# wsntxxn/AudioCaption

Measured on AMD Instinct MI355X. Metric: clips/sec (10 s @ 32 kHz) encode+greedy-decode, Cnn14_Rnn-Trm, higher is better.
Workload: dtype bf16x3

## Files before the change

### audiocaption_amd/csrc/conv3x3_block1_w4.hip

```cpp
#include <stdlib.h>
#include <string.h>
#include <type_traits>

#include "ac_common.h"
#include "ac_drop.h"
#include "ac_wino43.h"

namespace {

#ifndef B1_RING
#define B1_RING 3
#endif

#ifndef B1_RING_MFC
#define B1_RING_MFC 6
#endif
#ifndef B1_SGB_MEM
#define B1_SGB_MEM 0x0b0
#endif
#ifndef B1_SGB
#define B1_SGB 0
#endif
#ifndef B1_KO
#define B1_KO 0
#endif
#ifdef B1_CLK
__device__ unsigned long long b1_clk[8];
#endif

typedef unsigned u32x4 __attribute__((ext_vector_type(4)));

struct B1Params {
  const float* in;
  const float* w1;
  const float* sc1;
  const float* sh1;
  const void* wpk;
  const float* scale;
  const float* shift;
  float* out;
  int rows_total, Hp, H;
  int tiles;
  const int* clip_frames;
  int need_mul, need_add;
  Drop drop;
};

constexpr int B1_W = 64, B1_COLP = 3;
constexpr int B1_HALF = (((B1_W + 2) * B1_COLP * 16 + 127) / 128) * 128 + 64;
constexpr int B1_PLANE = 2 * B1_HALF;
constexpr int B1_VBUF = 12 * B1_PLANE;
constexpr int B1_WT = 2 * B1_VBUF;
constexpr int B1_LDS = B1_WT + 4096;
static_assert(B1_LDS <= 160 * 1024, "LDS");

template <int FORM, bool DROP>
__global__ __launch_bounds__(256, 1) void block1_w4_kernel(B1Params p) {
  constexpr bool FUSED = FORM == 1, MFC = FORM == 2;
  constexpr int HALF = B1_HALF, PLANE = B1_PLANE, VBUF = B1_VBUF, COLP = B1_COLP;
  extern __shared__ __attribute__((aligned(128))) unsigned char dsm_raw[];
  unsigned char* sV = dsm_raw;
  float* wt = (float*)(dsm_raw + B1_WT);
  const int tid = threadIdx.x;
  const int lane = tid & 63;
  const int wave = __builtin_amdgcn_readfirstlane(tid >> 6);
  const int half = lane >> 5;
  const int cg = wave & 1, wq = wave >> 1;
  const int nblk = (int)gridDim.x;

  auto tile_live = [&](int t) { return w4_rows_live(8 * t, 8, p.rows_total, p.Hp, p.H, p.clip_frames, p.need_mul, p.need_add); };
  auto zero_tile = [&](int t) {
    const f32x4 z = {0.f, 0.f, 0.f, 0.f};
    float* o = p.out + (size_t)t * 4 * 32 * 64;
    const long left = ((long)p.rows_total / 2 - 4L * t) * 32 * 64;
#pragma unroll
    for (int k = 0; k < 8; ++k) {
      const int i = (k * 256 + tid) * 4;
      if (i < left) *(f32x4*)(o + i) = z;
    }
  };
  auto next_live = [&](int t) {
    t += nblk;
    while (t < p.tiles && !tile_live(t)) { zero_tile(t); t += nblk; }
    return t;
  };
  int tile = next_live((int)blockIdx.x - nblk);
  if (tile >= p.tiles) return;

  {
    constexpr int NZ = 2 * 24 * 2 * COLP;
    const f32x4 z = {0.f, 0.f, 0.f, 0.f};
    for (int i = tid; i < NZ; i += 256) {
      const int slot = i % COLP, col = (i / COLP) & 1, hh = (i / (2 * COLP)) % 24, b = i / (48 * COLP);
      *(f32x4*)(sV + b * VBUF + hh * HALF + ((col ? B1_W + 1 : 0) * COLP + slot) * 16) = z;
    }
    if (FUSED) {
      for (int i = tid; i < 64 * 12; i += 256) {
        const int ch = i / 12, k = i % 12;
        wt[i] = k < 9 ? p.w1[ch * 9 + k] : (k == 9 ? p.sc1[ch] : (k == 10 ? p.sh1[ch] : 0.f));
      }
    }
    if (MFC && tid < 128) {
      const int ct = tid >> 6, l = tid & 63, ch = 32 * ct + (l & 31), h = l >> 5;
      const float sc = p.sc1[ch];
      f32x4 v[2];
#pragma unroll
      for (int q = 0; q < 8; ++q) {
        const int ky = 2 * h + q / 4, kx = q % 4;
        float w = 0.f;
        if (ky < 3 && kx < 3) w = p.w1[ch * 9 + ky * 3 + kx] * sc;
        if (ky == 3 && kx == 0) w = p.sh1[ch];
        v[q / 4][q % 4] = w;
      }
      u32x2 hi0, lo0, hi1, lo1;
      split_bf16x4(v[0], hi0, lo0);
      split_bf16x4(v[1], hi1, lo1);
      unsigned* dst = (unsigned*)(dsm_raw + B1_WT) + (ct * 2 * 64 + l) * 4;
      dst[0] = hi0.x; dst[1] = hi0.y; dst[2] = hi1.x; dst[3] = hi1.y;
      dst[256] = lo0.x; dst[257] = lo0.y; dst[258] = lo1.x; dst[259] = lo1.y;
    }
  }

  unsigned pb[2];
  {
    const int i = lane & 31;
#pragma unroll
    for (int m = 0; m < 2; ++m) pb[m] = (unsigned)(half * HALF + ((32 * m + i) * COLP + wq) * 16);
  }
  const int cq = tid & 3, scol = tid >> 2;
  unsigned lofs[2];
#pragma unroll
  for (int j = 0; j < 2; ++j) lofs[j] = (unsigned)((cq >> 1) * HALF + ((scol + 1) * COLP + j) * 16 + (cq & 1) * 8);

  const __amdgpu_buffer_rsrc_t rw = __builtin_amdgcn_make_buffer_rsrc((void*)p.wpk, 0, 4 * 18 * 4096, 0x00020000);
  const unsigned wvoff = (unsigned)(cg * 2048 + lane * 16);
  auto w_load = [&](int s, int gi, bf16x8 (&w)[2]) {
    const unsigned soff = (unsigned)((s & 3) * 18 + gi) * 4096u;
    w[0] = __builtin_bit_cast(bf16x8, __builtin_amdgcn_raw_buffer_load_b128(rw, wvoff, soff, 0));
    w[1] = __builtin_bit_cast(bf16x8, __builtin_amdgcn_raw_buffer_load_b128(rw, wvoff + 1024u, soff, 0));
  };

  const size_t in_elems = (size_t)p.rows_total * 64 * (FORM ? 1 : 64);
  const __amdgpu_buffer_rsrc_t rx = __builtin_amdgcn_make_buffer_rsrc(
      (void*)p.in, 0, (int)(in_elems * 4 < 0x7fffffffull ? in_elems * 4 : 0x7fffffffull), 0x00020000);

  auto load_x = [&](int t, float (&x)[12][3]) {
    const int cl = scol == 0 ? 0 : scol - 1, cr = scol == 63 ? 63 : scol + 1;
#pragma unroll
    for (int j = 0; j < 12; ++j) {
      const int gr = 8 * t - 2 + j;
      const unsigned off = (unsigned)(gr * 256);
      const float a = __builtin_bit_cast(float, __builtin_amdgcn_raw_buffer_load_b32(rx, off + (unsigned)(cl * 4), 0, 0));
      const float b = __builtin_bit_cast(float, __builtin_amdgcn_raw_buffer_load_b32(rx, off + (unsigned)(scol * 4), 0, 0));
      const float c = __builtin_bit_cast(float, __builtin_amdgcn_raw_buffer_load_b32(rx, off + (unsigned)(cr * 4), 0, 0));
      x[j][0] = scol == 0 ? 0.f : a;
      x[j][1] = b;
      x[j][2] = scol == 63 ? 0.f : c;
    }
  };
  float touch = 0.f;
  auto touch_x = [&](int t) {
    if (tid < 24) {
      const unsigned off = (unsigned)(((8 * t - 2) * 64 + tid * 32) * 4);
      touch = __builtin_bit_cast(float, __builtin_amdgcn_raw_buffer_load_b32(rx, off, 0, 0));
    }
  };
  auto row_mask = [&](int t) {
    unsigned m = 0;
    for (int r = 0; r < 10; ++r) {
      const int gr = 8 * t - 1 + r;
      if (gr >= 0 && gr < p.rows_total && (gr % p.Hp) < p.H) m |= 1u << r;
    }
    return m;
  };

  f32x16 acc[6][2];
  constexpr int RING = MFC && !DROP ? B1_RING_MFC : B1_RING, AH = RING - 1;
  bf16x8 wr[RING][2];
  bf16x8 af[2][2][2];
  float xc[12][3];
  unsigned mask_c = 0;
  f32x4 c1[10];
  f32x4 c1b[10];
  f32x4 w1r[4][3];

  auto conv1_row = [&](const float (&x)[12][3], unsigned mask, int r) {
    f32x4 y;
#pragma unroll
    for (int e = 0; e < 4; ++e) {
      float a = 0.f;
#pragma unroll
      for (int t = 0; t < 9; ++t) a = fmaf(x[r + t / 3][t % 3], w1r[e][t / 4][t % 4], a);
      y[e] = fmaxf(fmaf(a, w1r[e][2][1], w1r[e][2][2]), 0.f);
    }
    const f32x4 z = {0.f, 0.f, 0.f, 0.f};
    return (mask >> r) & 1u ? y : z;
  };
  auto taps_load = [&](int s) {
#pragma unroll
    for (int e = 0; e < 4; ++e)
#pragma unroll
      for (int k = 0; k < 3; ++k) w1r[e][k] = *(const f32x4*)(wt + ((s & 3) * 16 + cq * 4 + e) * 12 + 4 * k);
  };
  auto rows_request = [&](int t, int s, f32x4 (&dst)[10]) {
#pragma unroll
    for (int r = 0; r < 10; ++r) {
      const long gr = 8L * t - 1 + r;
      const unsigned off = (unsigned)(((gr * 64 + scol) * 64 + (s & 3) * 16 + cq * 4) * 4);
      dst[r] = __builtin_bit_cast(f32x4, __builtin_amdgcn_raw_buffer_load_b128(rx, off, 0, 0));
    }
  };
  auto piece = [&](unsigned char* buf, const f32x4 (&d)[10], int j, int pos) {
    const f32x4 v = w4_transform(pos, d[4 * j], d[4 * j + 1], d[4 * j + 2], d[4 * j + 3], d[4 * j + 4], d[4 * j + 5]);
    u32x2 hi, lo;
    split_bf16x4(v, hi, lo);
    unsigned char* dst = buf + lofs[j] + (2 * pos) * PLANE;
    *(u32x2*)dst = hi;
    *(u32x2*)(dst + PLANE) = lo;
  };
  auto stage_unit = [&](unsigned char* buf, int gi, int S, const float (&x)[12][3], unsigned mask, f32x4 (&d)[10]) {
    constexpr int ROW_AT[16] = {0, 1, 2, 3, 4, -1, -1, 5, -1, 6, 7, 8, -1, -1, 9, -1};
    constexpr int PIECE_AT[16] = {-1, -1, -1, -1, -1, 0, 2, -1, 4, -1, -1, -1, 6, 8, -1, 10};
    if (gi >= 16 || (B1_KO & 1)) return;
    if (FUSED && gi == 0) taps_load(S);
    if (FUSED && ROW_AT[gi] >= 0) d[ROW_AT[gi]] = conv1_row(x, mask, ROW_AT[gi]);
    if (PIECE_AT[gi] >= 0) {
      piece(buf, d, PIECE_AT[gi] / 6, PIECE_AT[gi] % 6);
      piece(buf, d, (PIECE_AT[gi] + 1) / 6, (PIECE_AT[gi] + 1) % 6);
    }
  };
  auto a_load = [&](const unsigned char* buf, int gi, bf16x8 (&a)[2][2]) {
    const int kx = gi / 6, q = gi % 6;
    const unsigned char* vh = buf + (2 * q) * PLANE + kx * COLP * 16;
#pragma unroll
    for (int m = 0; m < 2; ++m) {
      a[m][0] = *(const bf16x8*)(vh + pb[m]);
      a[m][1] = *(const bf16x8*)(vh + PLANE + pb[m]);
    }
  };

  const int m1 = wave & 1, j1 = wave >> 1;
  const int c1col = 32 * m1 + (lane & 31);
  unsigned lofs1[2];
#pragma unroll
  for (int gh = 0; gh < 2; ++gh) lofs1[gh] = (unsigned)(gh * HALF + ((c1col + 1) * COLP + j1) * 16 + half * 8);
  f32x4 xr[7];
  u32x2 rph[7], rpl[7];
  f32x4 d1[4][6];
  f32x16 c1a[2];
  bf16x8 a1h, a1l;
  auto x_request = [&](int t) {
    const int row0 = 8 * t - 2 + 4 * j1 + 2 * half;
    const int cadj = c1col == 0 ? 0 : c1col - 1;
#pragma unroll
    for (int k = 0; k < 7; ++k)
      xr[k] = __builtin_bit_cast(f32x4, __builtin_amdgcn_raw_buffer_load_b128(rx, (unsigned)(((row0 + k) * 64 + cadj) * 4), 0, 0));
  };
  auto x_convert = [&](int k) {
    const bool first = c1col == 0, last = c1col == 63;
    if (B1_KO & 64) {
      rph[k].x = __builtin_bit_cast(unsigned, xr[k][0]); rph[k].y = __builtin_bit_cast(unsigned, xr[k][1]);
      rpl[k].x = __builtin_bit_cast(unsigned, xr[k][2]); rpl[k].y = __builtin_bit_cast(unsigned, xr[k][3]);
      return;
    }
    const float e0 = first ? 0.f : xr[k][0], e1 = first ? xr[k][0] : xr[k][1];
    const float e2 = last ? 0.f : (first ? xr[k][1] : xr[k][2]);
    const unsigned h0 = cvt_pk_bf16(e0, e1), h1 = cvt_pk_bf16(e2, 0.f);
    const float f0 = __builtin_bit_cast(float, h0 << 16), f1 = __builtin_bit_cast(float, h0 & 0xffff0000u);
    const float f2 = __builtin_bit_cast(float, h1 << 16);
    rph[k].x = h0; rph[k].y = h1;
    rpl[k].x = cvt_pk_bf16(e0 - f0, e1 - f1);
    rpl[k].y = cvt_pk_bf16(e2 - f2, 0.f);
  };
  auto a1_load = [&](int ct) {
    const unsigned char* t = dsm_raw + B1_WT + (ct * 2 * 64 + lane) * 16;
    a1h = *(const bf16x8*)t;
    a1l = *(const bf16x8*)(t + 1024);
  };
  auto c1_mfma = [&](int which, int r) {
    f32x16& a = c1a[r & 1];
    if (B1_KO & 32) {
      if (which == 0) {
#pragma unroll
        for (int k = 0; k < 16; ++k) a[k] = __builtin_bit_cast(float, rph[r].x);
      } else {
        a[which] += __builtin_bit_cast(float, rpl[r + 1].y);
      }
      return;
    }
    if (which == 0) {
      const u32x4 bl = {rpl[r].x, rpl[r].y, half ? 0u : rpl[r + 1].x, half ? 0u : rpl[r + 1].y};
      f32x16 z;
#pragma unroll
      for (int k = 0; k < 16; ++k) z[k] = 0.f;
      a = __builtin_amdgcn_mfma_f32_32x32x16_bf16(a1h, __builtin_bit_cast(bf16x8, bl), z, 0, 0, 0);
    } else {
      const u32x4 bh = {rph[r].x, rph[r].y, half ? 0x3f80u : rph[r + 1].x, half ? 0u : rph[r + 1].y};
      a = __builtin_amdgcn_mfma_f32_32x32x16_bf16(which == 1 ? a1l : a1h, __builtin_bit_cast(bf16x8, bh), a, 0, 0, 0);
    }
  };
  auto c1_post = [&](int r, unsigned mask) {
    const float cap = (mask >> (4 * j1 + r)) & 1u ? __builtin_inff() : 0.f;
#pragma unroll
    for (int g = 0; g < 4; ++g)
#pragma unroll
      for (int e = 0; e < 4; ++e) d1[g][r][e] = __builtin_amdgcn_fmed3f(c1a[r & 1][4 * g + e], 0.f, cap);
  };
  auto piece1 = [&](unsigned char* buf, int g, int pos) {
    const f32x4 v = w4_transform(pos, d1[g][0], d1[g][1], d1[g][2], d1[g][3], d1[g][4], d1[g][5]);
    u32x2 hi, lo;
    split_bf16x4(v, hi, lo);
    unsigned char* dst = buf + lofs1[g & 1] + (2 * pos) * PLANE;
    if (B1_KO & 8) {
      asm volatile("" :: "v"(hi), "v"(lo), "v"(dst));
      return;
    }
    *(u32x2*)dst = hi;
    *(u32x2*)(dst + PLANE) = lo;
  };
  auto stage_a = [&](unsigned char* buf, int gi, int ct, unsigned mask) {
    if (B1_KO & 1) return;
    if (gi == 0) a1_load(ct);
    if (gi == 0) {
#pragma unroll
      for (int k = 0; k < 7; ++k) x_convert(k);
    }
    if (gi >= 2 && gi <= 7) c1_post(gi - 2, mask);
    if (gi >= 8 && gi <= 15 && !(B1_KO & 16)) {
      const int p0 = 3 * ((gi - 8) >> 1) + 2 * (gi & 1), np = gi & 1 ? 1 : 2;
#pragma unroll
      for (int q = p0; q < p0 + np; ++q) piece1(buf, q & 1, q >> 1);
    }
  };
  auto stage_b = [&](unsigned char* buf, int gi) {
    if (B1_KO & 1) return;
    if (gi < 12 && !(B1_KO & 16)) piece1(buf, 2 + (gi & 1), gi >> 1);
  };

  lds_barrier();
  static_assert(18 % RING == 0, "ring positions are static");
#pragma unroll
  for (int g0 = 0; g0 < AH; ++g0) w_load(0, g0, wr[g0]);
  if (FUSED) {
    load_x(tile, xc);
    mask_c = row_mask(tile);
  } else if (MFC) {
    x_request(tile);
    mask_c = row_mask(tile);
  } else {
    rows_request(tile, 0, c1);
    rows_request(tile, 1, c1b);
  }
  if (MFC) {
    a1_load(0);
#pragma unroll
    for (int k = 0; k < 7; ++k) x_convert(k);
#pragma unroll
    for (int r = 0; r < 6; ++r) {
#pragma unroll
      for (int k = 0; k < 3; ++k) c1_mfma(k, r);
      c1_post(r, mask_c);
    }
#pragma unroll
    for (int gi = 8; gi < 16; ++gi) stage_a(sV, gi, 0, mask_c);
  } else {
#pragma unroll
    for (int gi = 0; gi < 16; ++gi) stage_unit(sV, gi, 0, xc, mask_c, c1);
  }
  lds_barrier();
  a_load(sV, 0, af[0]);

  const __amdgpu_buffer_rsrc_t rsc = __builtin_amdgcn_make_buffer_rsrc((void*)p.scale, 0, 256, 0x00020000);
  const __amdgpu_buffer_rsrc_t rsh = __builtin_amdgcn_make_buffer_rsrc((void*)p.shift, 0, 256, 0x00020000);
  const FastDiv4 by_hp_out(p.Hp / 2);
  const int chw = cg * 32 + 4 * half;
  const f32x4 zero4 = {0.f, 0.f, 0.f, 0.f};

#ifdef B1_CLK
  unsigned long long clk_loop = 0, clk_epi = 0, clk_n = 0, clk_even = 0, clk_s1 = 0;
  const unsigned long long clk_t0 = __builtin_readcyclecounter(), clk_rt0 = __builtin_amdgcn_s_memrealtime();
#endif
#pragma unroll 1
  while (tile < p.tiles) {
#ifdef B1_CLK
    const unsigned long long clk_a = __builtin_readcyclecounter();
#endif
    const int next = next_live(tile);
    auto step = [&](auto S_) {
      constexpr int s = decltype(S_)::value;
      const unsigned char* cur = sV + (s & 1) * VBUF;
      unsigned char* nxt = sV + ((s + 1) & 1) * VBUF;
#pragma unroll
      for (int gi = 0; gi < 18; ++gi) {
        const int q = gi % 6;
        if (gi + 1 < 18) a_load(cur, gi + 1, af[(gi + 1) & 1]);
        else a_load(nxt, 0, af[0]);
        if (gi + AH < 18) w_load(s, gi + AH, wr[(gi + AH) % RING]);
        else w_load(s + 1, gi + AH - 18, wr[(gi + AH) % RING]);
        if (!(B1_KO & 2)) {
#pragma unroll
        for (int m = 0; m < 2; ++m) {
          if (s == 0 && gi < 6) {
            f32x16 z;
#pragma unroll
            for (int r = 0; r < 16; ++r) z[r] = 0.f;
            acc[q][m] = __builtin_amdgcn_mfma_f32_32x32x16_bf16(wr[gi % RING][0], af[gi & 1][m][1], z, 0, 0, 0);
          } else {
            acc[q][m] = __builtin_amdgcn_mfma_f32_32x32x16_bf16(wr[gi % RING][0], af[gi & 1][m][1], acc[q][m], 0, 0, 0);
          }
        }
        const bool C1ROW = MFC && (s & 1) && gi >= 1 && gi <= 6 && !(B1_KO & 1);
        if (C1ROW) c1_mfma(0, gi - 1);
#pragma unroll
        for (int m = 0; m < 2; ++m)
          acc[q][m] = __builtin_amdgcn_mfma_f32_32x32x16_bf16(wr[gi % RING][1], af[gi & 1][m][0], acc[q][m], 0, 0, 0);
        if (C1ROW) c1_mfma(1, gi - 1);
#pragma unroll
        for (int m = 0; m < 2; ++m)
          acc[q][m] = __builtin_amdgcn_mfma_f32_32x32x16_bf16(wr[gi % RING][0], af[gi & 1][m][0], acc[q][m], 0, 0, 0);
        if (C1ROW) c1_mfma(2, gi - 1);
        } else {
#pragma unroll
          for (int m = 0; m < 2; ++m)
            asm volatile("" :: "v"(af[gi & 1][m][0]), "v"(af[gi & 1][m][1]), "v"(wr[gi % RING][0]), "v"(wr[gi % RING][1]));
          if (s == 0 && gi < 6) {
#pragma unroll
            for (int m = 0; m < 2; ++m)
#pragma unroll
              for (int r = 0; r < 16; ++r) acc[q][m][r] = 0.f;
          }
        }
        if (MFC) {
          if (s & 1) stage_a(nxt, gi, s == 1 ? 1 : 0, mask_c);
          else stage_b(nxt, gi);
          if (!(s & 1) && gi == 13) x_request(s == 0 ? tile : next);
          if (s == 0 && gi == 16) touch_x(next);
          if (s == 2 && gi == 16) mask_c = row_mask(next);
        } else if (FUSED) {
          stage_unit(nxt, gi, s + 1, xc, mask_c, c1);
          if (s == 0 && gi == 16) touch_x(next);
          if (s == 2 && gi == 16) {
            load_x(next, xc);
            mask_c = row_mask(next);
          }
        } else {
          if (((s + 1) & 1) == 0) stage_unit(nxt, gi, s + 1, xc, mask_c, c1);
          else stage_unit(nxt, gi, s + 1, xc, mask_c, c1b);
          if (gi == 0) {
            const int t2 = s + 2 < 4 ? tile : next;
            if ((s & 1) == 0) rows_request(t2, s + 2, c1);
            else rows_request(t2, s + 2, c1b);
          }
        }
        if (gi == 16) lds_barrier();
        if (B1_SGB > 0 && MFC) {
#pragma unroll
          for (int i = 0; i < 9; ++i) {
            __builtin_amdgcn_sched_group_barrier(0x008, 1, 0);
            __builtin_amdgcn_sched_group_barrier(0x002, B1_SGB, 0);
            __builtin_amdgcn_sched_group_barrier(B1_SGB_MEM, 1, 0);
          }
        }
        __builtin_amdgcn_sched_barrier(0);
      }
    };
    step(std::integral_constant<int, 0>{});
#ifdef B1_CLK
    const unsigned long long clk_s0 = __builtin_readcyclecounter();
    clk_even += clk_s0 - clk_a;
#endif
    step(std::integral_constant<int, 1>{});
#ifdef B1_CLK
    clk_s1 += __builtin_readcyclecounter() - clk_s0;
#endif
    step(std::integral_constant<int, 2>{});
    step(std::integral_constant<int, 3>{});

#ifdef B1_CLK
    const unsigned long long clk_b = __builtin_readcyclecounter();
#endif
    {
      f32x4 sc4[4], sh4[4];
#pragma unroll
      for (int g = 0; g < 4; ++g) {
        sc4[g] = __builtin_bit_cast(f32x4, __builtin_amdgcn_raw_buffer_load_b128(rsc, (unsigned)(chw * 4 + 32 * g), 0, 0));
        sh4[g] = __builtin_bit_cast(f32x4, __builtin_amdgcn_raw_buffer_load_b128(rsh, (unsigned)(chw * 4 + 32 * g), 0, 0));
      }
      const int qg = 2 * tile + wq;
      const int hp0 = by_hp_out.mod(2 * qg);
      const long left = ((long)(p.rows_total / 2) - 4L * tile) * (32 * 64 * 4);
      const __amdgpu_buffer_rsrc_t ro = __builtin_amdgcn_make_buffer_rsrc(
          (void*)(p.out + (size_t)tile * (4 * 32 * 64)), 0, (int)(left < 32768 ? (left < 0 ? 0 : left) : 32768), 0x00020000);
#pragma unroll
      for (int m = 0; m < 2; ++m) {
        const int col = 32 * m + (lane & 31);
        const bool valid = hp0 + (col & 1) < p.H / 2;
        const unsigned ob = (unsigned)((((2 * wq + (col & 1)) * 32 + (col >> 1)) * 64 + chw) * 4);
#pragma unroll
        for (int g = 0; g < 4; ++g) {
          f32x4 t0, t1, o;
#pragma unroll
          for (int e = 0; e < 4; ++e) {
            const int r = 4 * g + e;
            float y[4];
            w4_outputs(acc[0][m][r], acc[1][m][r], acc[2][m][r], acc[3][m][r], acc[4][m][r], acc[5][m][r], sc4[g][e],
                       sh4[g][e], y);
            t0[e] = y[0] + y[1];
            t1[e] = y[2] + y[3];
          }
#pragma unroll
          for (int e = 0; e < 4; ++e) {
            const float a = t0[e] + dpp_mov<DPP_QUAD_XOR1>(t0[e]), b = t1[e] + dpp_mov<DPP_QUAD_XOR1>(t1[e]);
            o[e] = 0.25f * ((col & 1) ? b : a);
          }
          if (!valid) o = zero4;
          if (DROP) {
            const size_t oi = (size_t)tile * (4 * 32 * 64) + ob / 4 + 8 * g;
#pragma unroll
            for (int e = 0; e < 4; ++e) o[e] *= p.drop.mask(oi + e);
          }
          if (!(B1_KO & 4))
            __builtin_amdgcn_raw_buffer_store_b128(__builtin_bit_cast(u32x4, o), ro, ob + 32u * g, 0, 0);
        }
      }
    }
    asm volatile("" :: "v"(touch));
#ifdef B1_CLK
    clk_loop += clk_b - clk_a;
    clk_epi += __builtin_readcyclecounter() - clk_b;
    ++clk_n;
#endif
    tile = next;
  }
#ifdef B1_CLK
  if (tid == 0) {
    atomicAdd(&b1_clk[0], clk_loop);
    atomicAdd(&b1_clk[1], clk_epi);
    atomicAdd(&b1_clk[2], __builtin_readcyclecounter() - clk_t0);
    atomicAdd(&b1_clk[3], __builtin_amdgcn_s_memrealtime() - clk_rt0);
    atomicAdd(&b1_clk[4], clk_n);
    atomicAdd(&b1_clk[5], clk_even);
    atomicAdd(&b1_clk[6], clk_s1);
  }
#endif
}

template <int FORM, bool DROP>
int launch_b1(const B1Params& p, hipStream_t s) {
  static AcLdsAttr lds_attr;
  if (ac_allow_lds((const void*)block1_w4_kernel<FORM, DROP>, 160 * 1024, &lds_attr) != AC_OK) return AC_ERR_LAUNCH;
  static int cus_of[64];
  int dev = 0, cus = 0;
  if (hipGetDevice(&dev) != hipSuccess) return AC_ERR_LAUNCH;
  if (dev >= 0 && dev < 64) cus = __atomic_load_n(&cus_of[dev], __ATOMIC_RELAXED);
  if (!cus) {
    if (hipDeviceGetAttribute(&cus, hipDeviceAttributeMultiprocessorCount, dev) != hipSuccess) return AC_ERR_LAUNCH;
    if (cus <= 0) cus = 256;
    if (dev >= 0 && dev < 64) __atomic_store_n(&cus_of[dev], cus, __ATOMIC_RELAXED);
  }
  const unsigned grid = (unsigned)(p.tiles < cus ? p.tiles : cus);
  hipLaunchKernelGGL((block1_w4_kernel<FORM, DROP>), dim3(grid), dim3(256), (size_t)B1_LDS, s, p);
  return ac_check_launch();
}

}

static int b1_dispatch(int form, const float* in, const float* w1, const float* sc1, const float* sh1, const void* wfrag2,
                       const float* scale2, const float* shift2, float* out, int B, int Hp, int H, const int* clip_frames,
                       int need_mul, int need_add, void* stream, Drop drop) {
  if (!in || !wfrag2 || !scale2 || !shift2 || !out || (form && (!w1 || !sc1 || !sh1))) return AC_ERR_ARG;
  if (B <= 0 || Hp <= H || (Hp & 7) || H < 2) return AC_ERR_ARG;
  if (((unsigned long long)B * Hp + 4096) * 256 >= (1ull << 31)) return AC_ERR_ARG;
  if (!form && (unsigned long long)B * Hp * 64 * 64 * 4 >= (1ull << 31)) return AC_ERR_ARG;
  B1Params p;
  p.in = in; p.w1 = w1; p.sc1 = sc1; p.sh1 = sh1; p.wpk = wfrag2; p.scale = scale2; p.shift = shift2; p.out = out;
  p.rows_total = B * Hp; p.Hp = Hp; p.H = H;
  p.tiles = p.rows_total / 8;
  p.clip_frames = clip_frames; p.need_mul = need_mul; p.need_add = need_add;
  p.drop = drop;
  const hipStream_t st = (hipStream_t)stream;
  if (drop.thresh != 0) return form == 2 ? launch_b1<2, true>(p, st) : form == 1 ? launch_b1<1, true>(p, st) : AC_ERR_ARG;
  return form == 2 ? launch_b1<2, false>(p, st) : form == 1 ? launch_b1<1, false>(p, st) : launch_b1<0, false>(p, st);
}

#ifdef B1_CLK
extern "C" int ac_b1_clk_read(unsigned long long* out5, int reset) {
  if (hipMemcpyFromSymbol(out5, HIP_SYMBOL(b1_clk), 56) != hipSuccess) return -2;
  if (reset) { unsigned long long z[8] = {0, 0, 0, 0, 0, 0, 0, 0}; if (hipMemcpyToSymbol(HIP_SYMBOL(b1_clk), z, 64) != hipSuccess) return -2; }
  return 0;
}
#endif

extern "C" int ac_conv3x3_block1_wino43(const float* in1, const float* w1, const float* scale1, const float* shift1,
                                        const void* wfrag2, const float* scale2, const float* shift2, float* out, int B,
                                        int Hp, int H, const int* clip_frames, int need_mul, int need_add, float drop_p,
                                        unsigned long long drop_seed, const unsigned long long* seed_dev, void* stream) {
  if (!(drop_p >= 0.f) || drop_p >= 1.f) return AC_ERR_ARG;
  return b1_dispatch(1, in1, w1, scale1, shift1, wfrag2, scale2, shift2, out, B, Hp, H, clip_frames, need_mul, need_add,
                     stream, make_drop(drop_p, drop_seed, seed_dev));
}

extern "C" int ac_conv3x3_block1_wino43_mfma(const float* in1, const float* w1, const float* scale1, const float* shift1,
                                             const void* wfrag2, const float* scale2, const float* shift2, float* out, int B,
                                             int Hp, int H, const int* clip_frames, int need_mul, int need_add, float drop_p,
                                             unsigned long long drop_seed, const unsigned long long* seed_dev, void* stream) {
  if (!(drop_p >= 0.f) || drop_p >= 1.f) return AC_ERR_ARG;
  return b1_dispatch(2, in1, w1, scale1, shift1, wfrag2, scale2, shift2, out, B, Hp, H, clip_frames, need_mul, need_add,
                     stream, make_drop(drop_p, drop_seed, seed_dev));
}

extern "C" int ac_conv3x3_block1_conv2_wino43(const float* in64, const void* wfrag2, const float* scale2, const float* shift2,
                                              float* out, int B, int Hp, int H, void* stream) {
  return b1_dispatch(0, in64, nullptr, nullptr, nullptr, wfrag2, scale2, shift2, out, B, Hp, H, nullptr, 0, 0, stream,
                     make_drop(0.f, 0, nullptr));
}
```

Before: 15730.

## Switch block1 Winograd kernel to dynamic atomic tile scheduling

Replaces the static strided tile assignment in the persistent block1 conv kernel with a global atomic ticket counter per output buffer, so blocks pull the next tile on demand. Wave 0 resolves the next live tile mid-step, zeroes skipped dead tiles with buffer stores, and shares the result through LDS. The goal is better load balance when tile liveness varies per clip. It adds global atomics, a reset protocol that depends on a done counter, and a host-side slot table keyed by output pointer; the prefetch of the next tile's input is moved later to match.

```diff
diff --git a/audiocaption_amd/csrc/conv3x3_block1_w4.hip b/audiocaption_amd/csrc/conv3x3_block1_w4.hip
--- a/audiocaption_amd/csrc/conv3x3_block1_w4.hip
+++ b/audiocaption_amd/csrc/conv3x3_block1_w4.hip
@@ -24,9 +24,20 @@
 #ifndef B1_KO
 #define B1_KO 0
 #endif
+#ifndef B1_DYN
+#define B1_DYN 1
+#endif
 #ifdef B1_CLK
 __device__ unsigned long long b1_clk[8];
 #endif
+
+struct alignas(64) B1Slot {
+  unsigned ticket;
+  unsigned done;
+  unsigned pad[14];
+};
+constexpr int B1_SLOTS = 256, B1_SLOTS_USED = B1_SLOTS - 16;
+__device__ B1Slot b1_slots[B1_SLOTS];
 
 typedef unsigned u32x4 __attribute__((ext_vector_type(4)));
 
@@ -43,6 +54,7 @@
   int tiles;
   const int* clip_frames;
   int need_mul, need_add;
+  int slot;
   Drop drop;
 };
 
@@ -51,7 +63,8 @@
 constexpr int B1_PLANE = 2 * B1_HALF;
 constexpr int B1_VBUF = 12 * B1_PLANE;
 constexpr int B1_WT = 2 * B1_VBUF;
-constexpr int B1_LDS = B1_WT + 4096;
+constexpr int B1_NEXT = B1_WT + 4096;
+constexpr int B1_LDS = B1_NEXT + 16;
 static_assert(B1_LDS <= 160 * 1024, "LDS");
 
 template <int FORM, bool DROP>
@@ -69,23 +82,62 @@
   const int nblk = (int)gridDim.x;
 
   auto tile_live = [&](int t) { return w4_rows_live(8 * t, 8, p.rows_total, p.Hp, p.H, p.clip_frames, p.need_mul, p.need_add); };
-  auto zero_tile = [&](int t) {
-    const f32x4 z = {0.f, 0.f, 0.f, 0.f};
-    float* o = p.out + (size_t)t * 4 * 32 * 64;
-    const long left = ((long)p.rows_total / 2 - 4L * t) * 32 * 64;
-#pragma unroll
-    for (int k = 0; k < 8; ++k) {
-      const int i = (k * 256 + tid) * 4;
-      if (i < left) *(f32x4*)(o + i) = z;
-    }
-  };
-  auto next_live = [&](int t) {
-    t += nblk;
-    while (t < p.tiles && !tile_live(t)) { zero_tile(t); t += nblk; }
-    return t;
-  };
-  int tile = next_live((int)blockIdx.x - nblk);
+  auto zero_tile = [&](int t, int nthr, int me) {
+    const long left = ((long)(p.rows_total / 2) - 4L * t) * (32 * 64 * 4);
+    const __amdgpu_buffer_rsrc_t ro = __builtin_amdgcn_make_buffer_rsrc(
+        (void*)(p.out + (size_t)t * (4 * 32 * 64)), 0, (int)(left < 32768 ? (left < 0 ? 0 : left) : 32768), 0x00020000);
+    const u32x4 z = {0u, 0u, 0u, 0u};
+#pragma unroll 1
+    for (int i = me * 16; i < 32768; i += nthr * 16) __builtin_amdgcn_raw_buffer_store_b128(z, ro, (unsigned)i, 0, 0);
+  };
+  B1Slot* const sl = p.slot >= 0 ? &b1_slots[p.slot] : nullptr;
+  volatile int* const nx = (volatile int*)(dsm_raw + B1_NEXT);
+  auto draw_ask = [&]() { return atomicAdd(&sl->ticket, 1u); };
+  const __amdgpu_buffer_rsrc_t rsl = __builtin_amdgcn_make_buffer_rsrc((void*)(sl ? sl : b1_slots), 0, sl ? 4 : 0, 0x00020000);
+  auto draw_ask_quiet = [&](bool wanted) {
+    return (unsigned)__builtin_amdgcn_raw_ptr_buffer_atomic_add_i32(1, rsl, wanted ? tid * 4 : 1024, 0, 0);
+  };
+  auto draw_tile = [&](unsigned ticket) {
+    const unsigned t = ticket + (unsigned)nblk;
+    if (t < (unsigned)p.tiles) return (int)t;
+    if (atomicAdd(&sl->done, 1u) == (unsigned)nblk - 1u) {
+      atomicExch(&sl->ticket, 0u);
+      atomicExch(&sl->done, 0u);
+    }
+    return p.tiles;
+  };
+  unsigned ticket = 0;
+  auto next_live_wave0 = [&](int t, unsigned asked) {
+    const int ln = lane;
+    int c = 0;
+    if (sl) {
+      if (ln == 0) c = draw_tile(asked);
+      c = __builtin_amdgcn_readfirstlane(c);
+      while (c < p.tiles && !tile_live(c)) {
+        zero_tile(c, 64, ln);
+        if (ln == 0) c = draw_tile(draw_ask());
+        c = __builtin_amdgcn_readfirstlane(c);
+      }
+    } else {
+      c = t + nblk;
+      while (c < p.tiles && !tile_live(c)) { zero_tile(c, 64, ln); c += nblk; }
+    }
+    return c;
+  };
+  int tile = (int)blockIdx.x;
+  while (tile < p.tiles && !tile_live(tile)) {
+    zero_tile(tile, 256, tid);
+    if (wave == 0) {
+      int c = sl ? 0 : tile + nblk;
+      if (sl && lane == 0) c = draw_tile(draw_ask());
+      if (lane == 0) *nx = c;
+    }
+    lds_barrier();
+    tile = __builtin_amdgcn_readfirstlane(*nx);
+    lds_barrier();
+  }
   if (tile >= p.tiles) return;
+  if (sl && tid == 0) ticket = draw_ask();
 
   {
     constexpr int NZ = 2 * 24 * 2 * COLP;
@@ -385,7 +437,7 @@
 #ifdef B1_CLK
     const unsigned long long clk_a = __builtin_readcyclecounter();
 #endif
-    const int next = next_live(tile);
+    int next = p.tiles;
     auto step = [&](auto S_) {
       constexpr int s = decltype(S_)::value;
       const unsigned char* cur = sV + (s & 1) * VBUF;
@@ -434,11 +486,11 @@
           if (s & 1) stage_a(nxt, gi, s == 1 ? 1 : 0, mask_c);
           else stage_b(nxt, gi);
           if (!(s & 1) && gi == 13) x_request(s == 0 ? tile : next);
-          if (s == 0 && gi == 16) touch_x(next);
+          if (s == 1 && gi == 1) touch_x(next);
           if (s == 2 && gi == 16) mask_c = row_mask(next);
         } else if (FUSED) {
           stage_unit(nxt, gi, s + 1, xc, mask_c, c1);
-          if (s == 0 && gi == 16) touch_x(next);
+          if (s == 1 && gi == 1) touch_x(next);
           if (s == 2 && gi == 16) {
             load_x(next, xc);
             mask_c = row_mask(next);
@@ -452,7 +504,9 @@
             else rows_request(t2, s + 2, c1b);
           }
         }
+        if (s == 0 && gi == 16 && wave == 0) *nx = next_live_wave0(tile, ticket);
         if (gi == 16) lds_barrier();
+        if (s == 0 && gi == 16) next = __builtin_amdgcn_readfirstlane(*nx);
         if (B1_SGB > 0 && MFC) {
 #pragma unroll
           for (int i = 0; i < 9; ++i) {
@@ -486,6 +540,7 @@
         sc4[g] = __builtin_bit_cast(f32x4, __builtin_amdgcn_raw_buffer_load_b128(rsc, (unsigned)(chw * 4 + 32 * g), 0, 0));
         sh4[g] = __builtin_bit_cast(f32x4, __builtin_amdgcn_raw_buffer_load_b128(rsh, (unsigned)(chw * 4 + 32 * g), 0, 0));
       }
+      ticket = draw_ask_quiet(next < p.tiles);
       const int qg = 2 * tile + wq;
       const int hp0 = by_hp_out.mod(2 * qg);
       const long left = ((long)(p.rows_total / 2) - 4L * tile) * (32 * 64 * 4);
@@ -543,6 +598,24 @@
     atomicAdd(&b1_clk[6], clk_s1);
   }
 #endif
+}
+
+int b1_slot_of(int dev, const void* out) {
+  struct Table { const void* key[B1_SLOTS_USED]; int n; };
+  static Table tables[64];
+  static int lock;
+  if (dev < 0 || dev >= 64) return -1;
+  Table& t = tables[dev];
+  while (__atomic_exchange_n(&lock, 1, __ATOMIC_ACQUIRE)) {}
+  int slot = -1;
+  for (int i = 0; i < t.n && slot < 0; ++i)
+    if (t.key[i] == out) slot = i;
+  if (slot < 0 && t.n < B1_SLOTS_USED) {
+    slot = t.n++;
+    t.key[slot] = out;
+  }
+  __atomic_store_n(&lock, 0, __ATOMIC_RELEASE);
+  return slot;
 }
 
 template <int FORM, bool DROP>
@@ -559,7 +632,9 @@
     if (dev >= 0 && dev < 64) __atomic_store_n(&cus_of[dev], cus, __ATOMIC_RELAXED);
   }
   const unsigned grid = (unsigned)(p.tiles < cus ? p.tiles : cus);
-  hipLaunchKernelGGL((block1_w4_kernel<FORM, DROP>), dim3(grid), dim3(256), (size_t)B1_LDS, s, p);
+  B1Params q = p;
+  q.slot = B1_DYN && (unsigned)p.tiles > grid ? b1_slot_of(dev, p.out) : -1;
+  hipLaunchKernelGGL((block1_w4_kernel<FORM, DROP>), dim3(grid), dim3(256), (size_t)B1_LDS, s, q);
   return ac_check_launch();
 }
 
@@ -577,6 +652,7 @@
   p.rows_total = B * Hp; p.Hp = Hp; p.H = H;
   p.tiles = p.rows_total / 8;
   p.clip_frames = clip_frames; p.need_mul = need_mul; p.need_add = need_add;
+  p.slot = -1;
   p.drop = drop;
   const hipStream_t st = (hipStream_t)stream;
   if (drop.thresh != 0) return form == 2 ? launch_b1<2, true>(p, st) : form == 1 ? launch_b1<1, true>(p, st) : AC_ERR_ARG;
```

Result: no change. 15640 (-0.6%).
